# vt-asaplab/vPIN

Measured on AMD Instinct MI355X. Metric: R1CS constraints/sec, whole Spartan SNARK (sat proof + SPARK evaluation proof; vPIN point-mult + point-add instances), higher is better.
Workload: dtype u256 (integers mod q and mod p = 2^255-19, 32-bit limbs); 1 GPU; vPIN LeNet trace (layers L1..L7): 12 SNARKs per step; inputs=resident in HBM, parallelism=one trace per rank x 1 rank(s), no collective; 4 stream(s) per rank, table_slot_bytes=128

## Files before the change

### include/vpin_hip.h

```cpp
#ifndef VPIN_HIP_H
#define VPIN_HIP_H
#include <stddef.h>
#include <stdint.h>

#ifdef __cplusplus
extern "C" {
#endif

#define VPIN_OK 0
#define VPIN_EINVAL (-1)
#define VPIN_ENODEV (-2)
#define VPIN_ENOMEM (-3)
#define VPIN_EHIP (-4)
#define VPIN_ESHAPE (-5)
#define VPIN_EVERIFY (-6)

typedef struct vpin_ctx vpin_ctx;
typedef struct vpin_table vpin_table;

const char* vpin_strerror(int code);
const char* vpin_last_error(void);
int vpin_crash_line_set(const char* line, size_t n);
int vpin_abi_version(void);

// ... 559 lines not shown

int vpin_bullet_reduce(vpin_ctx* c, const vpin_gens* g, const uint8_t* x_mont, const uint8_t* a_mont, size_t R, const uint8_t* u_mont,
                       int classic, uint8_t* cLR_out, uint8_t* LR_out, uint8_t xhat_ahat_out[64], uint8_t ghat_out[32]);

int vpin_gadget_shape(int is_mult, size_t n_ops, size_t* num_cons, size_t* num_vars, size_t nnz[3]);
size_t vpin_gadget_proof_max_bytes(int is_mult, size_t n_ops);
size_t vpin_gadget_comm_bytes(int is_mult, size_t n_ops);
size_t vpin_gadget_vars_rows(int is_mult, size_t n_ops);
int vpin_host_gens_derive(const char* label, size_t nb, uint8_t* out_xyzt );
int vpin_host_merlin_kat(const char* proto, const char* label, const uint8_t* msg, size_t n, const char* clabel,
                         uint8_t* out, size_t out_n);
int vpin_host_commit(const char* label, const uint8_t* v_mont, size_t n, const uint8_t* blind_mont, uint8_t out[32]);

int vpin_host_scalar_mul2(const uint8_t a_mont[32], const uint8_t P[32], const uint8_t b_mont[32], const uint8_t Q[32], uint8_t out[32]);

int vpin_host_eq_round(const uint8_t* rand, int k, int npc, int with_dotp, int lead, const uint8_t* claims, const uint8_t* coeffs,
                       const uint8_t* res, const uint8_t* r, uint8_t* polys_out, uint8_t* state_out);

int vpin_host_mailbox_selftest(void);

#define VPIN_K_SC_CUBIC 0
#define VPIN_K_SC_QUAD 1
#define VPIN_K_SC_BIND 2
#define VPIN_K_SC_CUBIC_FUSED 3
#define VPIN_K_SC_QUAD_FUSED 4
#define VPIN_K_EQ 5
#define VPIN_K_MSM 6
#define VPIN_K_SC_TAIL 7
#define VPIN_K_SPARK_ROUND 8
#define VPIN_K_SPARK_BUILD 9
#define VPIN_K_SPARK_ROUND_BIG 10
#define VPIN_K_MSM_ROWS 11
#define VPIN_K_SPARK_TAIL 12
#define VPIN_K_COUNT 16
typedef struct {
  uint64_t launches;
  double ms;
  double alg_bytes;
  double units;
} vpin_kstat;
int vpin_prof_enable(vpin_ctx* ctx, int on);
int vpin_prof_reset(vpin_ctx* ctx);
int vpin_prof_read(vpin_ctx* ctx, vpin_kstat* stats);

#ifdef __cplusplus
}
#endif
#endif
```

### vpin_amd/capi.py

```python
import ctypes as C
import os
import re

import numpy as np

HERE = os.path.dirname(os.path.abspath(__file__))
ROOT = os.path.dirname(HERE)
HEADER = os.path.join(ROOT, "include", "vpin_hip.h")

KERNEL_CLASSES = {
    0: "sc_cubic", 1: "sc_quad", 2: "sc_bind", 3: "sc_cubic_fused", 4: "sc_quad_fused", 5: "eq", 6: "msm", 7: "sc_tail",
    8: "spark_round", 9: "spark_build", 10: "spark_round_big", 11: "msm_rows", 12: "spark_tail",
}
K_COUNT = 16


class VpinError(RuntimeError):
    def __init__(self, code, where):
        self.code = code
        L = lib()
        msg = L.vpin_strerror(code).decode()
        last = L.vpin_last_error().decode()
        super().__init__(f"{where}: {msg} ({code})" + (f" [{last}]" if last else ""))


class R1CS(C.Structure):
    _fields_ = [("num_cons", C.c_size_t), ("num_vars", C.c_size_t), ("num_inputs", C.c_size_t),
                ("nnz", C.c_size_t * 3), ("row", C.c_void_p * 3), ("col", C.c_void_p * 3), ("val", C.c_void_p * 3)]


def make_r1cs(inst):
    r = R1CS()
    r.num_cons, r.num_vars, r.num_inputs = inst["num_cons"], inst["num_vars"], inst["num_inputs"]
    keep = []
    for m, name in enumerate("ABC"):
        rows, cols, vals = (np.ascontiguousarray(x) for x in inst[name])
        keep += [rows, cols, vals]
        r.nnz[m] = len(rows)
        r.row[m] = rows.ctypes.data
        r.col[m] = cols.ctypes.data
        r.val[m] = vals.ctypes.data
    r._keep = keep
    return r


# ... 1607 lines not shown
```

### vpin_amd/csrc/host/prover_common.h

```cpp
#pragma once
#include <omp.h>

#include <chrono>
#include <cstdlib>
#include <cstring>
#include <map>
#include <memory>
#include <mutex>
#include <string>
#include <vector>

#include "../ctx.h"
#include "../comm.h"
#include "curve.h"
#include "transcript.h"

extern "C" {
size_t vpin_gens_msm_parts_count(size_t ncols);
int vpin_gens_msm_parts(vpin_ctx* ctx, const vpin_gens* g, const uint8_t* scalars_mont, size_t rows, size_t ncols,
                        uint8_t* parts_xyzt);
int vpin_poly_bound(vpin_ctx* c, const vpin_table* Z, const uint8_t* Lvec, size_t L_size, uint8_t* out_LZ);
int vpin_gens_map_stream(vpin_ctx* ctx, const uint8_t* stream64, size_t nb, uint8_t* out_xyzt);
void vpin_r1cs_dims(const vpin_r1cs_dev* d, size_t* num_cons, size_t* num_vars, size_t* num_inputs);
}
// ... 418 lines not shown
  if (fine)
    fprintf(stderr, "[dplog] R=%zu, %zu rounds, us per round: rows+inner products %.1f | host Q,H terms %.1f | wait for the MSM %.1f | "
            "sum %zu parts x2 %.1f | compress x2 + transcript + invert %.1f | fold launch %.1f\n", R, lgR, tb[0] / lgR * 1e6,
            tb[1] / lgR * 1e6, tb[2] / lgR * 1e6, np, tb[3] / lgR * 1e6, tb[4] / lgR * 1e6, tb[5] / lgR * 1e6);
  Fq xa[2];
  if (fused) rc = vpin::bullet_finish_fused(c, pc.dev, bs, B(&u_prev), B(&u_inv_prev), B(xa));
  else rc = vpin::bullet_finish(c, pc.dev, bs, B(xa), parts.data());
  if (rc) return rc;
  const Fq x_hat = xa[0], a_hat = xa[1], y_hat = x_hat * a_hat;
  Point g_hat = fused ? sum_side(0, 0) : sum_parts(parts.data());
  {
    Point p = g_hat.mul(d_);
    pc.fb_h.mul_acc(p, r_delta);
    out.delta = compress(p);
    tr.append_point("delta", out.delta.b);
    Point q = pc.fb_gR.mul(d_ * r_);
    pc.fb_h.mul_acc(q, r_beta);
    out.beta = compress(q);
    tr.append_point("beta", out.beta.b);
  }
  Fq c_ = tr.challenge_scalar("c");
  out.z1 = d_ + c_ * y_hat;
  out.z2 = a_hat * (c_ * blind_fin + r_beta) + r_delta;
  bs_guard.done = true;
  return VPIN_OK;
}

struct TableGuard {
  vpin_ctx* c;
  std::vector<vpin_table*> t;
  explicit TableGuard(vpin_ctx* c_) : c(c_) {}
  ~TableGuard() { for (auto* p : t) vpin_table_free(c, p); }
  vpin_table* add(vpin_table* p) { t.push_back(p); return p; }
};

#if defined(__clang__)
#pragma clang diagnostic pop
#endif

int sat_prove_core(vpin_ctx* c, const vpin_r1cs_dev* dinst, size_t nv, size_t ncons, size_t ni,
                   const vpin_table* d_para, const vpin_table* d_input, const vpin_table* d_vars, const uint8_t* inputs,
                   const uint8_t seed_commit64[64], const uint8_t seed_proof64[64], uint8_t* proof_out, size_t proof_cap,
                   size_t* proof_len, uint8_t* comm_para_out, uint8_t* comm_input_out, uint8_t inst_evals_out[96],
                   uint8_t* rx_out, uint8_t* ry_out, vpin_host::Transcript* tr_out, vpin_host::Transcript* tape_out);

}
```

### vpin_amd/csrc/prover.cpp

```cpp
#include "host/proof_sizes.h"
#include "host/prover_common.h"

namespace {

using namespace vpin_host;
using namespace vpin_prover;


struct SatGens {
  size_t ell = 0, L = 0, R = 0, nb = 0;
  std::vector<Point> g;
  FixedBase fb[5];
  const vpin_gens* dev = nullptr;
  PcGens pc;
  Mcg gens_1, gens_3, gens_4;
};

struct ProverCache {
  std::map<size_t, std::unique_ptr<SatGens>> by_nv;
};

static void cache_free(vpin_ctx* c) {
  auto* pc = static_cast<ProverCache*>(c->prover_cache);
  if (!pc) return;
// ... 419 lines not shown

namespace vpin_prover {

static int dist_fingerprint_check(vpin_ctx* c, size_t nv, size_t ncons, size_t ni, const uint8_t seed_commit64[64],
                                  const uint8_t seed_proof64[64]) {
  vpin_comm* cm = c->comm;
  auto fnv = [](const uint8_t* p, size_t n) { uint64_t h = 0xcbf29ce484222325ull; for (size_t i = 0; i < n; i++) { h ^= p[i]; h *= 0x100000001b3ull; } return h; };
  auto env_num = [](const char* name, long dflt) { const char* e = getenv(name); return e ? atol(e) : dflt; };
  uint64_t fp[9] = {
      (uint64_t)nv, (uint64_t)ncons, (uint64_t)ni, fnv(seed_commit64, 64), fnv(seed_proof64, 64),
      (uint64_t)(getenv("VPIN_DIST_NO_SAT_SPLIT") != nullptr), (uint64_t)(getenv("VPIN_DIST_BY_CIRCUIT") != nullptr),
      (uint64_t)env_num("VPIN_SPARK_TAIL_PAIRS", 1024), (uint64_t)(getenv("VPIN_BULLET_CLASSIC") != nullptr)};
  std::vector<uint64_t> all((size_t)cm->world * 9);
  int rc = vpin::comm_allgather_ctx(c, fp, all.data(), sizeof fp, "fingerprint");
  if (rc) return rc;
  static const char* what[9] = {"num_vars", "num_cons", "num_inputs", "seed_commit", "seed_proof", "VPIN_DIST_NO_SAT_SPLIT",
                                "VPIN_DIST_BY_CIRCUIT", "VPIN_SPARK_TAIL_PAIRS", "VPIN_BULLET_CLASSIC"};
  for (int r = 0; r < cm->world; r++)
    for (int k = 0; k < 9; k++)
      if (all[(size_t)r * 9 + k] != fp[k]) {
        char msg[200];
        snprintf(msg, sizeof msg, "collective proof: rank %d and rank %d differ in %s (%llu vs %llu)", cm->rank, r, what[k],
                 (unsigned long long)fp[k], (unsigned long long)all[(size_t)r * 9 + k]);
        vpin::set_last_error(msg, hipErrorUnknown);
        return VPIN_ECOMM;
      }
  return VPIN_OK;
}

int sat_prove_core(vpin_ctx* c, const vpin_r1cs_dev* dinst, size_t nv, size_t ncons, size_t ni,
                   const vpin_table* d_para, const vpin_table* d_input, const vpin_table* d_vars, const uint8_t* inputs,
                   const uint8_t seed_commit64[64], const uint8_t seed_proof64[64], uint8_t* proof_out, size_t proof_cap,
                   size_t* proof_len, uint8_t* comm_para_out, uint8_t* comm_input_out, uint8_t inst_evals_out[96],
                   uint8_t* rx_out, uint8_t* ry_out, vpin_host::Transcript* tr_out, vpin_host::Transcript* tape_out) {
  auto t_begin = Clock::now();
  memset(g_timings, 0, sizeof g_timings);
  (void)hipSetDevice(c->device);

  SatGens* sg = nullptr;
  auto t0 = Clock::now();
  int rc = get_gens(c, nv, &sg);
  if (rc) return rc;
  g_timings[5] = secs(t0, Clock::now());
  const size_t L = sg->L, R = sg->R;
  TableGuard tg(c);

  t0 = Clock::now();
  vpin_comm* cm = (c->comm && c->comm->world > 1) ? c->comm : nullptr;
  if (cm && (rc = dist_fingerprint_check(c, nv, ncons, ni, seed_commit64, seed_proof64))) return rc;
  const size_t nrows = cm ? vpin::comm_strided_count(L, cm->rank, cm->world) : L;
  vpin::CommitPairState* cps = nullptr;
  if (nrows && (rc = vpin::commit_pair_begin(c, sg->dev, d_para, d_input, L, &cps, cm ? (size_t)cm->rank : 0, nrows, cm ? (size_t)cm->world : 1)))
    return rc;
  const uint8_t two = 2;
  Transcript tape1 = make_tape(&two, 1, seed_commit64);
  std::vector<Fq> blind_para = tape1.challenge_vector("poly_blinds", L);
  std::vector<Fq> blind_input = tape1.challenge_vector("poly_blinds", L);
  std::vector<Fq> blind_vars(L);
  for (size_t i = 0; i < L; i++) blind_vars[i] = blind_para[i] + blind_input[i];
  std::vector<CG> comm_vars(L);
  if (!cm) {
    rc = vpin::commit_pair_finish(c, sg->dev, cps, B(blind_para.data()), B(blind_input.data()), R + 1, comm_para_out,
                                  comm_input_out, comm_vars[0].b);
    if (rc) return rc;
  } else {
    const size_t pmax = vpin::comm_block_max(L, cm->world);
    std::vector<uint8_t> mine(3 * pmax * 32, 0), all((size_t)cm->world * 3 * pmax * 32);
// ... 57 lines not shown
  vpin_table* tabs1[3] = {d_abc[0], d_abc[1], d_abc[2]};
  rc = zk_sumcheck(c, 4, tabs1, Fq::zero(), Fq::zero(), nrx, sg->gens_1, sg->gens_4, tr, tape, sc1, rx, claims1, blind_post1,
                   &tau, d_pyr, lw);
  if (rc) return rc;
  if ((rc = vpin::comm_mark(c, "sat_phase1_rest"))) return rc;
  vpin::ctx_enter_alt(c);
  if (c->progress_flag) *c->progress_flag = 1;
  g_timings[1] = secs(t0, Clock::now());

  const Fq tau_claim = claims1[0], Az_claim = claims1[1], Bz_claim = claims1[2], Cz_claim = claims1[3];
  Fq Az_blind = tape.challenge_scalar("Az_blind"), Bz_blind = tape.challenge_scalar("Bz_blind"),
     Cz_blind = tape.challenge_scalar("Cz_blind"), prod_blind = tape.challenge_scalar("prod_Az_Bz_blind");
  KnowProof pok_Cz;
  CG comm_Cz = knowledge_prove(pok_Cz, sg->gens_1, tr, tape, Cz_claim, Cz_blind);
  ProdProof pprod;
  CG comm_Az, comm_Bz, comm_prod;
  product_prove(pprod, sg->gens_1, tr, tape, Az_claim, Az_blind, Bz_claim, Bz_blind, Az_claim * Bz_claim, prod_blind, comm_Az,
                comm_Bz, comm_prod);
  tr.append_point("comm_Az_claim", comm_Az.b);
  tr.append_point("comm_Bz_claim", comm_Bz.b);
  tr.append_point("comm_Cz_claim", comm_Cz.b);
  tr.append_point("comm_prod_Az_Bz_claims", comm_prod.b);
  Fq blind_expected1 = tau_claim * (prod_blind - Cz_blind);
  Fq claim_post1 = (Az_claim * Bz_claim - Cz_claim) * tau_claim;
  EqProof eq1;
  equality_prove(eq1, sg->gens_1, tr, tape, claim_post1, blind_expected1, claim_post1, blind_post1);

  t0 = Clock::now();
  Fq r_A = tr.challenge_scalar("challenege_Az"), r_B = tr.challenge_scalar("challenege_Bz"),
     r_C = tr.challenge_scalar("challenege_Cz");
  Fq claim2 = r_A * Az_claim + r_B * Bz_claim + r_C * Cz_claim;
  Fq blind_claim2 = r_A * Az_blind + r_B * Bz_blind + r_C * Cz_blind;
  vpin_table *d_eq_rx = nullptr, *d_eabc = nullptr;
  if ((rc = vpin_eq_table(c, B(rx.data()), nrx, &d_eq_rx))) return rc;
  tg.add(d_eq_rx);
  t_spmv = Clock::now();
  {
    Fq rabc[3] = {r_A, r_B, r_C};
    if (lw) rc = vpin::r1cs_eval_table_strided(c, dinst, d_eq_rx, B(rabc), wrank, wstep, &d_eabc);
    else rc = vpin_r1cs_eval_table(c, dinst, d_eq_rx, B(rabc), &d_eabc);
    if (rc) return rc;
    tg.add(d_eabc);
  }
  g_timings[6] += secs(t_spmv, Clock::now());
  Fq claims2[2], blind_post2;
  vpin_table* d_z2 = d_z;
  if (lw) {
    if ((rc = vpin::table_take_strided(c, d_z, wrank, wstep, &d_z2))) return rc;
    tg.add(d_z2);
  }
  vpin_table* tabs2[2] = {d_z2, d_eabc};
  rc = zk_sumcheck(c, 2, tabs2, claim2, blind_claim2, nry, sg->gens_1, sg->gens_3, tr, tape, sc2, ry, claims2, blind_post2, nullptr,
                   nullptr, lw);
  if (rc) return rc;
  if ((rc = vpin::comm_mark(c, "sat_phase2_rest"))) return rc;
  g_timings[2] = secs(t0, Clock::now());

  t0 = Clock::now();
  const size_t left = sg->ell / 2, right = sg->ell - left;
  std::vector<Fq> Lv(L), Rv(R), LZ(R);
  host_eq(ry.data() + 1, left, Lv.data());
  host_eq(ry.data() + 1 + left, right, Rv.data());
  if (cm) rc = vpin::poly_bound_dist(c, d_vars, B(Lv.data()), L, B(LZ.data()));
  else rc = vpin_poly_bound(c, d_vars, B(Lv.data()), L, B(LZ.data()));
  if (rc) return rc;
  Fq eval_vars_at_ry = Fq::zero();
  for (size_t i = 0; i < R; i++) eval_vars_at_ry = eval_vars_at_ry + LZ[i] * Rv[i];
  Fq blind_eval = tape.challenge_scalar("blind_eval");
  tr.append_protocol_name("polynomial evaluation proof");
  Fq LZ_blind = Fq::zero();
  for (size_t i = 0; i < L; i++) LZ_blind = LZ_blind + blind_vars[i] * Lv[i];

  DpLog pe;
  if ((rc = dplog_prove(c, sg->pc, tr, tape, LZ, LZ_blind, Rv, eval_vars_at_ry, blind_eval, pe))) return rc;
  g_timings[3] = secs(t0, Clock::now());

  Fq blind_eval_Z = (one - ry[0]) * blind_eval;
  Fq blind_expected2 = claims2[1] * blind_eval_Z;
  Fq claim_post2 = claims2[0] * claims2[1];
  EqProof eq2;
  equality_prove(eq2, sg->gens_1, tr, tape, claim_post2, blind_expected2, claim_post2, blind_post2);

  t0 = Clock::now();
  Fq ie[3];
  {
    vpin_table* d_eq_ry = nullptr;
    if ((rc = vpin_eq_table(c, B(ry.data()), nry, &d_eq_ry))) return rc;
    tg.add(d_eq_ry);
    if ((rc = vpin_r1cs_evaluate(c, dinst, d_eq_rx, d_eq_ry, B(ie)))) return rc;
  }
  tr.append_scalar("Ar_claim", ie[0]);
  tr.append_scalar("Br_claim", ie[1]);
  tr.append_scalar("Cr_claim", ie[2]);
  memcpy(inst_evals_out, ie, 96);
  g_timings[7] = secs(t0, Clock::now());

  Writer w;
  w.u64(L);
  for (auto& cg : comm_vars) w.point(cg);
  write_zksc(w, sc1);
  w.point(comm_Az); w.point(comm_Bz); w.point(comm_Cz); w.point(comm_prod);
  w.point(pok_Cz.alpha); w.scalar(pok_Cz.z1); w.scalar(pok_Cz.z2);
  w.point(pprod.alpha); w.point(pprod.beta); w.point(pprod.delta);
  for (int i = 0; i < 5; i++) w.scalar(pprod.z[i]);
  w.point(eq1.alpha); w.scalar(eq1.z);
  write_zksc(w, sc2);
  w.point(pe.Cy);
  write_dplog(w, pe);
  w.point(eq2.alpha); w.scalar(eq2.z);
  if (w.buf.size() > proof_cap) return VPIN_ESHAPE;
  memcpy(proof_out, w.buf.data(), w.buf.size());
  *proof_len = w.buf.size();
  if (rx_out) memcpy(rx_out, rx.data(), rx.size() * 32);
  if (ry_out) memcpy(ry_out, ry.data(), ry.size() * 32);
  if ((rc = vpin::comm_mark(c, "sat_replicated"))) return rc;
  if (tr_out) *tr_out = tr;
  if (tape_out) *tape_out = tape;
  g_timings[4] = secs(t_begin, Clock::now());
// ... 83 lines not shown
```

### vpin_amd/csrc/r1cs.hip

```cpp
#include <algorithm>
#include <cstring>
#include <vector>

#include "ctx.h"
#include "r1cs_dev.h"

namespace vpin {

constexpr int kRB = 256;

__device__ __forceinline__ fq mul_special(const fq& val, const fq& x) {
  return fq_mul(val, x);
}

__global__ __launch_bounds__(kRB) void spmv_kernel(const uint32_t* __restrict__ rowptr, const uint32_t* __restrict__ col,
                                                   const fq* __restrict__ val, const fq* __restrict__ z, size_t nrows,
                                                   fq* __restrict__ out) {
  size_t r = (size_t)blockIdx.x * kRB + threadIdx.x;
  if (r >= nrows) return;
  uint32_t k0 = rowptr[r], k1 = rowptr[r + 1];
  fq acc = fq_zero();
  for (uint32_t k = k0; k < k1; k++) {
    fq x = fq_load(z + col[k]);
    if (fq_is_zero(x)) continue;
// ... 557 lines not shown
    if (d->n_long[m]) {
      hipLaunchKernelGGL(long_chunk_kernel, dim3((unsigned)d->n_chunks[m]), dim3(kRB), 0, c->stream, d->chunk_k0[m],
                         d->chunk_k1[m], d->csc_row[m], d->csc_val[m], evals_rx->d, chunk_partials);
      hipLaunchKernelGGL(eval_table_long_finish_strided_kernel, dim3((unsigned)d->n_long[m]), dim3(64), 0, c->stream,
                         d->long_cols[m], d->long_first[m], d->n_long[m], chunk_partials, rc_m, r0, step, t->d);
    }
  }
  hipError_t e = hipGetLastError();
  if (e != hipSuccess) { set_last_error("eval_table_strided", e); vpin_table_free(c, t); return VPIN_EHIP; }
  *out = t;
  return VPIN_OK;
}

}

extern "C" {

int vpin_r1cs_evaluate(vpin_ctx* c, const vpin_r1cs_dev* d, const vpin_table* evals_rx, const vpin_table* evals_ry,
                       uint8_t out[96]) {
  if (!c || !d || !evals_rx || !evals_ry || !out) return VPIN_EINVAL;
  if (evals_rx->len != d->num_cons || evals_ry->len != 2 * d->num_vars) return VPIN_ESHAPE;
  (void)hipSetDevice(c->device);
  const size_t ncols = 2 * d->num_vars;
  DevBuf bo(c), chunk_scratch(c);
  if (bo.alloc(96)) return VPIN_ENOMEM;
  fq* d_out = (fq*)bo.p;
  const size_t max_chunks = std::max(d->n_chunks[0], std::max(d->n_chunks[1], d->n_chunks[2]));
  if (max_chunks && chunk_scratch.alloc(max_chunks * sizeof(fq))) return VPIN_ENOMEM;
  fq* chunk_partials = (fq*)chunk_scratch.p;
  int grid = (int)std::min<size_t>((ncols + kRB - 1) / kRB, 1024);
  for (int m = 0; m < 3; m++) {
    int nparts = grid + (int)d->n_long[m];
    if ((size_t)nparts > c->partials_cap) return VPIN_ESHAPE;
    hipLaunchKernelGGL(evaluate_kernel, dim3(grid), dim3(kRB), 0, c->stream, d->colptr[m], d->csc_row[m], d->csc_val[m],
                       evals_rx->d, evals_ry->d, ncols, c->d_partials);
    if (d->n_long[m]) {
      hipLaunchKernelGGL(long_chunk_kernel, dim3((unsigned)d->n_chunks[m]), dim3(kRB), 0, c->stream, d->chunk_k0[m],
                         d->chunk_k1[m], d->csc_row[m], d->csc_val[m], evals_rx->d, chunk_partials);
      hipLaunchKernelGGL(evaluate_long_finish_kernel, dim3((unsigned)d->n_long[m]), dim3(64), 0, c->stream,
                         d->long_cols[m], d->long_first[m], d->n_long[m], chunk_partials, evals_ry->d, c->d_partials + grid);
    }
    hipLaunchKernelGGL(sum_partials_kernel, dim3(1), dim3(kRB), 0, c->stream, c->d_partials, nparts, d_out + m);
  }
  hipError_t e = hipGetLastError();
  if (e == hipSuccess) e = hipMemcpyAsync(out, d_out, 96, hipMemcpyDeviceToHost, c->stream);
  if (e == hipSuccess) e = hipStreamSynchronize(c->stream);
  if (e != hipSuccess) { set_last_error("vpin_r1cs_evaluate", e); return VPIN_EHIP; }
  return VPIN_OK;
}

}
```

### vpin_amd/csrc/spark.cpp

```cpp
#include <cstdio>

#include "host/proof_sizes.h"
#include "host/prover_common.h"
#include "gadget_dev.h"
#include "spark_dev.h"

namespace {

using namespace vpin_host;
using namespace vpin_prover;

static bool spark_trace() { static const bool on = getenv("VPIN_SPARK_TRACE") != nullptr; return on; }
struct TraceSpan {
  const char* name; Clock::time_point t0;
  explicit TraceSpan(const char* n) : name(n), t0(Clock::now()) {}
  ~TraceSpan() { if (spark_trace()) fprintf(stderr, "[spark] %-28s %8.3f ms\n", name, secs(t0, Clock::now()) * 1e3); }
};


struct SparkGens {
  std::vector<Point> g;
  std::map<size_t, std::unique_ptr<PcGens>> views;
};

// ... 595 lines not shown
}

struct SparkProof {
  vpin_ctx* c;
  const vpin_spark_decomm* d;
  const std::vector<Fq>&rx, &ry;
  const Fq* evals;
  Transcript &tr, &tape;
  const size_t N, M, lgN, lgM;
  const PcGens *g_ops = nullptr, *g_mem = nullptr, *g_derefs = nullptr;
  TableGuard tg;
  DistPlan plan;
  const DistPlan* dz = nullptr;
  bool st = false;
  vpin::SparkLeaves leaves;
  size_t Nf = 0, Mf = 0;
  bool defer_mem = false;
  vpin_table *mem_rx = nullptr, *mem_ry = nullptr, *comb = nullptr;
  vpin_table comb_shape;
  vpin::DevBuf b_cloc, b_crows, b_vloc, b_ops, b_mem, b_scr;
  vpin::fq* comb_rows = nullptr;
  const vpin::fq *derefs = nullptr, *vals = nullptr;
  std::vector<CG> comm_derefs;
  vpin::HashParams hash;
  vpin::SparkForest f_ops, f_mem;
  Fq pl[2][8];
  DotpCtx dotp;
  Fq dotp_left[3], dotp_right[3];
  Batched pf_ops, pf_mem;
  std::vector<Fq> rand_ops, rand_mem;
  Fq ev_derefs[6], ev_ops[15], ev_mem[2];
  DpLog pe_derefs, pe_ops, pe_mem;

  SparkProof(vpin_ctx* c_, const vpin_spark_decomm* d_, const std::vector<Fq>& rx_, const std::vector<Fq>& ry_, const Fq* evals_,
             Transcript& tr_, Transcript& tape_)
      : c(c_), d(d_), rx(rx_), ry(ry_), evals(evals_), tr(tr_), tape(tape_), N(d_->N), M(d_->M), lgN(log2z(d_->N)), lgM(log2z(d_->M)),
        tg(c_), b_cloc(c_), b_crows(c_), b_vloc(c_), b_ops(c_), b_mem(c_), b_scr(c_) {}
  bool by_circuit() const { return dz && !st; }
};

static int split_plan(SparkProof& S) {
  vpin_ctx* c = S.c;
  if (!(c->comm && c->comm->world > 1)) return VPIN_OK;
  if (c->comm->world > 12) return VPIN_EINVAL;
  plan_init(S.plan, c->comm);
  S.dz = &S.plan;
  static const bool by_circuit = getenv("VPIN_DIST_BY_CIRCUIT") != nullptr;
  const size_t Wz = (size_t)S.plan.world;
  if (!by_circuit && (Wz & (Wz - 1)) == 0 && Wz <= 16 && S.N / Wz >= 4096 && S.M / Wz >= 4096 && S.g_derefs->L >= Wz)
    S.plan.lw = (int)log2z(Wz);
  S.st = S.plan.lw > 0;
  if (S.st) { S.leaves.r0 = (size_t)S.plan.rank; S.leaves.step = Wz; }
  return VPIN_OK;
}

static int stage_derefs(SparkProof& S) {
  vpin_ctx* c = S.c;
  const vpin_spark_decomm* d = S.d;
  const DistPlan* dz = S.dz;
  const PcGens* g_derefs = S.g_derefs;
  const size_t N = S.N;
  int rc;
  S.tr.append_protocol_name("Sparse polynomial evaluation proof");
  const size_t nm = std::max(d->nx, d->ny);
  std::vector<Fq> rx_ext(nm, Fq::zero()), ry_ext(nm, Fq::zero());
  std::copy(S.rx.begin(), S.rx.end(), rx_ext.begin() + (nm - d->nx));
  std::copy(S.ry.begin(), S.ry.end(), ry_ext.begin() + (nm - d->ny));
  if ((rc = vpin_eq_table(c, B(rx_ext.data()), (int)nm, &S.mem_rx))) return rc;
  S.tg.add(S.mem_rx);
  if ((rc = vpin_eq_table(c, B(ry_ext.data()), (int)nm, &S.mem_ry))) return rc;
  S.tg.add(S.mem_ry);
  const vpin::fq *mem_rx = S.mem_rx->d, *mem_ry = S.mem_ry->d;
  S.Nf = N / S.leaves.step; S.Mf = S.M / S.leaves.step;
  if (S.st) {
    S.comb_shape.d = nullptr; S.comb_shape.len = S.comb_shape.cap = 8 * N; S.comb_shape.owned = false;
    S.comb = &S.comb_shape;
    const size_t Nl = S.Nf, nrows_loc = vpin::comm_strided_count(g_derefs->L, dz->rank, dz->world);
    if (S.b_cloc.alloc(6 * Nl * 32) || S.b_crows.alloc(std::max<size_t>(1, nrows_loc) * g_derefs->R * 32) || S.b_vloc.alloc(3 * Nl * 32)) return VPIN_ENOMEM;
    S.comb_rows = (vpin::fq*)S.b_crows.p;
    if ((rc = vpin::spark_gather_derefs(c, d, S.leaves, mem_rx, mem_ry, (vpin::fq*)S.b_cloc.p, S.comb_rows, g_derefs->R, nrows_loc))) return rc;
    for (int m = 0; m < 3; m++)
      if ((rc = vpin::spark_take_strided(c, d->vals + (size_t)m * N, Nl, S.leaves.r0, S.leaves.step, (vpin::fq*)S.b_vloc.p + (size_t)m * Nl))) return rc;
    S.derefs = (const vpin::fq*)S.b_cloc.p; S.vals = (const vpin::fq*)S.b_vloc.p;
  } else {
    if ((rc = vpin::table_alloc_uninit(c, 8 * N, &S.comb))) return rc;
    S.tg.add(S.comb);
    if ((rc = vpin::spark_gather_derefs(c, d, S.leaves, mem_rx, mem_ry, S.comb->d))) return rc;
    S.derefs = S.comb->d; S.vals = d->vals;
  }
  if ((rc = vpin::comm_mark(c, "derefs_gather"))) return rc;
  std::vector<CG>& comm_derefs = S.comm_derefs;
  const bool hot = d->hot_col[0] != 0xffffffffu || d->hot_col[1] != 0xffffffffu || d->hot_col[2] != 0xffffffffu;
  const uint32_t* col_idx[3] = {d->idx + 6 * N, d->idx + 7 * N, d->idx + 8 * N};
  if (dz) {
    const size_t L = g_derefs->L, pmax = vpin::comm_block_max(L, dz->world);
    const size_t nrows = vpin::comm_strided_count(L, dz->rank, dz->world);
    std::vector<uint8_t> mine(pmax * 32, 0), all(pmax * 32 * (size_t)dz->world);
    if (nrows) {
      if (hot)
        rc = vpin::hyrax_commit_derefs_hot(c, g_derefs->dev, S.comb, L, N, col_idx, d->hot_col, mem_ry, mine.data(), (size_t)dz->rank,
                                           nrows, (size_t)dz->world, S.comb_rows);
      else
        rc = vpin::hyrax_commit_rows_strided(c, g_derefs->dev, S.comb, L, (size_t)dz->rank, nrows, (size_t)dz->world, mine.data(), S.comb_rows);
      if (rc) return rc;
    }
    if ((rc = vpin::comm_allgather_ctx(c, mine.data(), all.data(), mine.size(), "derefs_commit"))) return rc;
    comm_derefs.resize(L);
    for (int r = 0; r < dz->world; r++) {
      const size_t n = vpin::comm_strided_count(L, r, dz->world);
      for (size_t k = 0; k < n; k++) memcpy(comm_derefs[(size_t)r + k * (size_t)dz->world].b, all.data() + ((size_t)r * pmax + k) * 32, 32);
    }
  } else if (hot) {
    comm_derefs.resize(g_derefs->L);
    if ((rc = vpin::hyrax_commit_derefs_hot(c, g_derefs->dev, S.comb, g_derefs->L, N, col_idx, d->hot_col, mem_ry, comm_derefs[0].b))) return rc;
  } else if ((rc = commit_noblind(c, g_derefs, S.comb, comm_derefs))) {
    return rc;
  }
  S.tr.append_message("derefs_commitment", "begin_derefs_commitment");
  append_polycomm(S.tr, "comm_poly_row_col_ops_val", comm_derefs);
  S.tr.append_message("derefs_commitment", "end_derefs_commitment");
  return VPIN_OK;
}

// ... 76 lines not shown
      if (S.defer_mem) {
        if ((rc = vpin::spark_mem_roots(c, S.d, S.hash, S.mem_rx->d, S.mem_ry->d))) return rc;
      } else if (S.f_mem.ncirc && (rc = vpin::spark_fetch_tops(c, &S.f_mem, 2))) {
        return rc;
      }
      t = reinterpret_cast<const Fq*>(c->h_spark);
      if (dz) {
        if ((rc = dist_exchange(c, *dz, true, false, t, 2, roots.data(), "roots"))) return rc;
        t = roots.data();
      }
    }
    for (int s = 0; s < 2; s++) { pl[s][0] = t[2 * (2 * s)]; pl[s][7] = t[2 * (2 * s + 1)]; }
  }
  static const char* lab[2][4] = {{"claim_row_eval_init", "claim_row_eval_read", "claim_row_eval_write", "claim_row_eval_audit"},
                                  {"claim_col_eval_init", "claim_col_eval_read", "claim_col_eval_write", "claim_col_eval_audit"}};
  for (int s = 0; s < 2; s++) {
    Fq ws = Fq::one(), rs = Fq::one();
    for (int m = 0; m < 3; m++) { rs = rs * pl[s][1 + m]; ws = ws * pl[s][4 + m]; }
    if (!(pl[s][0] * ws == rs * pl[s][7])) return VPIN_ESHAPE;
    S.tr.append_scalar(lab[s][0], pl[s][0]);
    S.tr.append_scalars(lab[s][1], &pl[s][1], 3);
    S.tr.append_scalars(lab[s][2], &pl[s][4], 3);
    S.tr.append_scalar(lab[s][3], pl[s][7]);
  }
  return VPIN_OK;
}

static int dotp_claims(SparkProof& S) {
  vpin_ctx* c = S.c;
  const DistPlan* dz = S.dz;
  int rc;
  const std::vector<int>* hv = S.by_circuit() ? &dz->dotp_of[dz->rank] : nullptr;
  const size_t nh = hv ? hv->size() : 6;
  if (nh && (rc = vpin::spark_triple_sums(c, S.derefs, S.vals, S.Nf, hv ? hv->data() : nullptr, (int)nh))) return rc;
  Fq mine6[6] = {};
  for (size_t i = 0; i < nh; i++) mine6[hv ? (*hv)[i] : i] = reinterpret_cast<const Fq*>(c->h_spark)[3 * i];
  if (S.st) rc = dist_sum(c, *dz, mine6, 6, S.dotp.claims, "triple_sums");
  else if (dz) rc = dist_pick(c, *dz, mine6, 6, dz->owner_dotp, S.dotp.claims, "triple_sums");
  else std::copy(mine6, mine6 + 6, S.dotp.claims);
  if (rc) return rc;
  for (int m = 0; m < 3; m++) {
    S.dotp_left[m] = S.dotp.claims[2 * m];
    S.dotp_right[m] = S.dotp.claims[2 * m + 1];
    S.tr.append_scalar("claim_eval_dotp_left", S.dotp_left[m]);
    S.tr.append_scalar("claim_eval_dotp_right", S.dotp_right[m]);
    if (!(S.dotp_left[m] + S.dotp_right[m] == S.evals[m])) return VPIN_ESHAPE;
  }
  return VPIN_OK;
}

static int stage_product(SparkProof& S) {
  vpin_ctx* c = S.c;
  int rc;
  S.tr.append_protocol_name("Sparse polynomial evaluation proof");
  S.tr.append_protocol_name("Sparse polynomial product layer proof");
  if ((rc = product_roots(S))) return rc;
  S.dotp = DotpCtx{S.d, S.Nf, S.vals, S.derefs, (vpin::fq*)S.b_scr.p, {}};
  if ((rc = dotp_claims(S))) return rc;
  {
    TraceSpan ts("product: ops forest");
    if ((rc = product_prove(c, S.f_ops, 12, &S.dotp, S.tr, S.pf_ops, S.rand_ops, S.dz))) return rc;
  }
  if (S.defer_mem) {
    TraceSpan ts("network: mem forest (deferred)");
    S.b_ops.release();
    S.b_scr.release();
    if (S.b_mem.alloc((size_t)4 * 2 * S.M * 32)) return VPIN_ENOMEM;
    S.f_mem.base = (vpin::fq*)S.b_mem.p;
    if ((rc = vpin::spark_build_forest(c, S.d, S.hash, S.leaves, {nullptr, S.mem_rx->d, S.mem_ry->d}, &S.f_mem, true))) return rc;
// ... 130 lines not shown
    if ((rc = vpin::spark_slice_evals(c, comb_ops->d, N, 15, eq_ops->d))) return rc;
    for (int i = 0; i < 15; i++) S.ev_ops[i] = hs[3 * i];
    if ((rc = vpin::spark_slice_evals(c, comb_mem->d, M, 2, eq_mem->d))) return rc;
    for (int i = 0; i < 2; i++) S.ev_mem[i] = hs[3 * i];
  }
  std::vector<Fq> e16(16, Fq::zero());
  std::copy(S.ev_ops, S.ev_ops + 15, e16.begin());
  if ((rc = prove_joint(S, *S.g_ops, comb_ops, sp_ops, e16, 4, rand_ops,
                        {"claim_evals_ops", "challenge_combine_n_to_one", "joint_claim_eval_ops", "hash: polyeval ops"}, nullptr, S.pe_ops)))
    return rc;
  return prove_joint(S, *S.g_mem, comb_mem, sp_mem, {S.ev_mem[0], S.ev_mem[1]}, 1, rand_mem,
                     {"claim_evals_mem", "challenge_combine_two_to_one", "joint_claim_eval_mem", "hash: polyeval mem"}, nullptr, S.pe_mem);
}

static void write_proof(const SparkProof& S, Writer& w) {
  const auto& pl = S.pl;
  w.u64(S.comm_derefs.size());
  for (auto& p : S.comm_derefs) w.point(p);
  for (int s = 0; s < 2; s++) { w.scalar(pl[s][0]); w_scalars(w, &pl[s][1], 3); w_scalars(w, &pl[s][4], 3); w.scalar(pl[s][7]); }
  w_scalars(w, S.dotp_left, 3);
  w_scalars(w, S.dotp_right, 3);
  write_batched(w, S.pf_mem);
  write_batched(w, S.pf_ops);
  w_scalars(w, &S.ev_ops[0], 3); w_scalars(w, &S.ev_ops[3], 3); w.scalar(S.ev_mem[0]);
  w_scalars(w, &S.ev_ops[6], 3); w_scalars(w, &S.ev_ops[9], 3); w.scalar(S.ev_mem[1]);
  w_scalars(w, &S.ev_ops[12], 3);
  w_scalars(w, &S.ev_derefs[0], 3); w_scalars(w, &S.ev_derefs[3], 3);
  write_dplog(w, S.pe_ops);
  write_dplog(w, S.pe_mem);
  write_dplog(w, S.pe_derefs);
}

static int spark_prove(vpin_ctx* c, const vpin_spark_decomm* d, const std::vector<Fq>& rx, const std::vector<Fq>& ry,
                       const Fq evals[3], Transcript& tr, Transcript& tape, Writer& w) {
  if (d->N < 4 || d->M < 4 || rx.size() != d->nx || ry.size() != d->ny) return VPIN_ESHAPE;
  int rc;
  SparkProof S(c, d, rx, ry, evals, tr, tape);
  const Shape sh{d->nx, d->ny, S.N, S.M, S.lgN + 4, std::max(d->nx, d->ny) + 1, S.lgN + 3};
  if ((rc = get_view(c, std::max(sh.v_ops, sh.v_mem), &S.g_ops)) || (rc = get_view(c, sh.v_ops, &S.g_ops)) ||
      (rc = get_view(c, sh.v_mem, &S.g_mem)) || (rc = get_view(c, sh.v_derefs, &S.g_derefs)))
    return rc;
  auto t0 = Clock::now();
  auto lap = [&](int slot) { g_spark_timings[slot] = secs(t0, Clock::now()); t0 = Clock::now(); };
  if ((rc = split_plan(S)) || (rc = stage_derefs(S))) return rc;
  lap(1);
  if (c->progress_flag) *c->progress_flag = 2;
  if ((rc = stage_network(S))) return rc;
  lap(2);
  if ((rc = stage_product(S))) return rc;
  lap(3);
  if ((rc = stage_hash(S))) return rc;
  lap(4);
  write_proof(S, w);
  return VPIN_OK;
}

}

extern "C" {

size_t vpin_spark_comm_bytes(const vpin_r1cs* inst) {
  return inst ? vpin_sizes::spark_comm_bytes(inst->num_cons, inst->num_vars, inst->nnz) : 0;
}

size_t vpin_snark_proof_max_bytes(const vpin_r1cs* inst) {
  return inst ? vpin_sizes::snark_proof_max_bytes(inst->num_cons, inst->num_vars, inst->nnz) : 0;
}

int vpin_spark_prepare(vpin_ctx* c, size_t num_cons, size_t num_vars, size_t max_nnz) {
  if (!c || !vpin::is_pow2(num_cons) || !vpin::is_pow2(num_vars) || max_nnz == 0) return VPIN_EINVAL;
  (void)hipSetDevice(c->device);
  const size_t nnz[3] = {max_nnz, max_nnz, max_nnz};
  const Shape s = shape_of(num_cons, num_vars, nnz);
  const PcGens* g = nullptr;
  int rc = get_view(c, std::max(s.v_ops, s.v_mem), &g);
  if (!rc) {
    auto* sg = static_cast<SparkGens*>(c->spark_cache);
    std::vector<size_t> idx;
    for (size_t ell : {s.v_ops, s.v_mem, s.v_derefs}) {
      const size_t R = (size_t)1 << (ell - ell / 2);
      if (R + 1 < sg->g.size()) { idx.push_back(R); idx.push_back(R + 1); }
    }
#pragma omp parallel for schedule(dynamic, 1) num_threads(host_threads())
    for (long k = 0; k < (long)idx.size(); k++) { FixedBase warm(sg->g[idx[(size_t)k]]); (void)warm; }
  }
  if (!rc) rc = get_view(c, s.v_ops, &g);
// ... 199 lines not shown
  memcpy(rand.data(), r, r_len * 32);
  SlicePass sp(c);
  std::vector<Fq> ev((size_t)used);
  int rc = sp.run(c, pc, (const uint32_t*)b32.p, n32, used > n32 ? Zfq->d : nullptr, nbits, used, rand, ev.data());
  if (rc) return rc;
  memcpy(evals_out, ev.data(), (size_t)used * 32);
  if (ch && LZ_out) {
    std::vector<Fq> chv((size_t)nbits), LZ;
    memcpy(chv.data(), ch, (size_t)nbits * 32);
    if ((rc = sp.combine(c, pc, chv, LZ))) return rc;
    memcpy(LZ_out, LZ.data(), pc.R * 32);
  }
  return VPIN_OK;
}

int vpin_snark_prove_resident(vpin_ctx* c, const vpin_r1cs_dev* dinst, const vpin_spark_decomm* decomm,
                              const vpin_table* vars_para, const vpin_table* vars_input, const vpin_table* vars,
                              const uint8_t* inputs, const uint8_t seed_commit64[64], const uint8_t seed_proof64[64],
                              uint8_t* proof_out, size_t proof_cap, size_t* proof_len, uint8_t* comm_para_out,
                              uint8_t* comm_input_out) {
  if (!c || !dinst || !decomm || !vars_para || !vars_input || !vars || !seed_commit64 || !seed_proof64 || !proof_out ||
      !proof_len || !comm_para_out || !comm_input_out)
    return VPIN_EINVAL;
  size_t nv, ncons, ni;
  vpin_r1cs_dims(dinst, &ncons, &nv, &ni);
  if (vars_para->len != nv || vars_input->len != nv || vars->len != nv || (ni && !inputs)) return VPIN_ESHAPE;
  if (decomm->num_cons != ncons || decomm->num_vars != nv || decomm->num_inputs != ni) return VPIN_ESHAPE;
  auto t0 = Clock::now();
  vpin::AltStreamGuard alt_guard(c);
  Transcript tr("snark_example"), tape("snark_example");
  uint8_t ie[96];
  std::vector<Fq> rx(log2z(ncons)), ry(log2z(2 * nv));
  size_t sat_len = 0;
  int rc = sat_prove_core(c, dinst, nv, ncons, ni, vars_para, vars_input, vars, inputs, seed_commit64, seed_proof64, proof_out,
                          proof_cap, &sat_len, comm_para_out, comm_input_out, ie, B(rx.data()), B(ry.data()), &tr, &tape);
  if (rc) return vpin::comm_leave(c->comm, rc);
  if (c->progress_flag) *c->progress_flag = 1;
  g_spark_timings[5] = secs(t0, Clock::now());
  Writer w;
  w.bytes(ie, 96);
  Fq evals[3];
  memcpy(evals, ie, 96);
  if ((rc = spark_prove(c, decomm, rx, ry, evals, tr, tape, w))) return vpin::comm_leave(c->comm, rc);
  if (sat_len + w.buf.size() > proof_cap) return VPIN_ESHAPE;
  memcpy(proof_out + sat_len, w.buf.data(), w.buf.size());
  *proof_len = sat_len + w.buf.size();
  g_spark_timings[6] = secs(t0, Clock::now());
  return VPIN_OK;
}

int vpin_snark_prove(vpin_ctx* c, const vpin_r1cs* inst, const uint8_t* vars_para, const uint8_t* vars_input,
                     const uint8_t* vars, const uint8_t* inputs, const uint8_t seed_commit64[64], const uint8_t seed_proof64[64],
                     uint8_t* proof_out, size_t proof_cap, size_t* proof_len, uint8_t* comm_out, size_t comm_cap, size_t* comm_len,
                     uint8_t* comm_para_out, uint8_t* comm_input_out) {
  if (!c || !inst || !vars_para || !vars_input || !vars) return VPIN_EINVAL;
  const size_t nv = inst->num_vars;
  if (!vpin::is_pow2(nv) || !vpin::is_pow2(inst->num_cons) || inst->num_inputs >= nv) return VPIN_ESHAPE;
  vpin_r1cs_dev* dinst = nullptr;
  vpin_spark_decomm* decomm = nullptr;
  const bool trace = getenv("VPIN_CLI_TRACE") != nullptr;
  auto t0 = std::chrono::steady_clock::now();
  auto lap = [&](const char* what) {
    if (!trace) return;
    (void)hipStreamSynchronize(c->stream);
    auto t1 = std::chrono::steady_clock::now();
    fprintf(stderr, "[vpin_snark_prove] %-18s %9.1f ms\n", what, std::chrono::duration<double, std::milli>(t1 - t0).count());
    t0 = t1;
  };
  int rc = vpin_r1cs_upload(c, inst, &dinst);
  if (rc) return rc;
  lap("r1cs_upload");
  TableGuard tg(c);
  vpin_table *d_para = nullptr, *d_input = nullptr, *d_vars = nullptr;
  rc = vpin_spark_encode(c, inst, &decomm, comm_out, comm_cap, comm_len);
  lap("spark_encode");
  if (!rc) rc = vpin_table_upload(c, vars_para, nv, &d_para);
// ... 34 lines not shown
```

Before: 78.19 million constraints/s.

## Compute inst evals via SPARK deref gather, reusing eq tables across sat and SPARK

```diff
diff --git a/include/vpin_hip.h b/include/vpin_hip.h
--- a/include/vpin_hip.h
+++ b/include/vpin_hip.h
@@ -615,6 +615,7 @@
 #define VPIN_K_SPARK_ROUND_BIG 10
 #define VPIN_K_MSM_ROWS 11
 #define VPIN_K_SPARK_TAIL 12
+#define VPIN_K_R1CS_EVALUATE 13
 #define VPIN_K_COUNT 16
 typedef struct {
   uint64_t launches;
diff --git a/vpin_amd/capi.py b/vpin_amd/capi.py
--- a/vpin_amd/capi.py
+++ b/vpin_amd/capi.py
@@ -11,6 +11,7 @@
 KERNEL_CLASSES = {
     0: "sc_cubic", 1: "sc_quad", 2: "sc_bind", 3: "sc_cubic_fused", 4: "sc_quad_fused", 5: "eq", 6: "msm", 7: "sc_tail",
     8: "spark_round", 9: "spark_build", 10: "spark_round_big", 11: "msm_rows", 12: "spark_tail",
+    13: "r1cs_evaluate",
 }
 K_COUNT = 16
 
diff --git a/vpin_amd/csrc/host/prover_common.h b/vpin_amd/csrc/host/prover_common.h
--- a/vpin_amd/csrc/host/prover_common.h
+++ b/vpin_amd/csrc/host/prover_common.h
@@ -474,7 +474,21 @@
   explicit TableGuard(vpin_ctx* c_) : c(c_) {}
   ~TableGuard() { for (auto* p : t) vpin_table_free(c, p); }
   vpin_table* add(vpin_table* p) { t.push_back(p); return p; }
+  void release_all_but(vpin_table* keep) {
+    for (auto* p : t)
+      if (p != keep) vpin_table_free(c, p);
+    t.clear();
+  }
 };
+
+struct SparkPrelude {
+  const vpin_spark_decomm* d = nullptr;
+  vpin_table *mem_rx = nullptr, *mem_ry = nullptr, *comb = nullptr;
+  Fq sums[6];
+  bool done = false;
+  size_t nm() const;
+};
+int spark_prelude(vpin_ctx* c, SparkPrelude& P, const std::vector<Fq>& rx, const std::vector<Fq>& ry, vpin_table* eq_rx);
 
 #if defined(__clang__)
 #pragma clang diagnostic pop
@@ -484,6 +498,7 @@
                    const vpin_table* d_para, const vpin_table* d_input, const vpin_table* d_vars, const uint8_t* inputs,
                    const uint8_t seed_commit64[64], const uint8_t seed_proof64[64], uint8_t* proof_out, size_t proof_cap,
                    size_t* proof_len, uint8_t* comm_para_out, uint8_t* comm_input_out, uint8_t inst_evals_out[96],
-                   uint8_t* rx_out, uint8_t* ry_out, vpin_host::Transcript* tr_out, vpin_host::Transcript* tape_out);
-
-}
+                   uint8_t* rx_out, uint8_t* ry_out, vpin_host::Transcript* tr_out, vpin_host::Transcript* tape_out,
+                   SparkPrelude* pre = nullptr);
+
+}
diff --git a/vpin_amd/csrc/prover.cpp b/vpin_amd/csrc/prover.cpp
--- a/vpin_amd/csrc/prover.cpp
+++ b/vpin_amd/csrc/prover.cpp
@@ -475,7 +475,8 @@
                    const vpin_table* d_para, const vpin_table* d_input, const vpin_table* d_vars, const uint8_t* inputs,
                    const uint8_t seed_commit64[64], const uint8_t seed_proof64[64], uint8_t* proof_out, size_t proof_cap,
                    size_t* proof_len, uint8_t* comm_para_out, uint8_t* comm_input_out, uint8_t inst_evals_out[96],
-                   uint8_t* rx_out, uint8_t* ry_out, vpin_host::Transcript* tr_out, vpin_host::Transcript* tape_out) {
+                   uint8_t* rx_out, uint8_t* ry_out, vpin_host::Transcript* tr_out, vpin_host::Transcript* tape_out,
+                   SparkPrelude* pre) {
   auto t_begin = Clock::now();
   memset(g_timings, 0, sizeof g_timings);
   (void)hipSetDevice(c->device);
@@ -599,8 +600,21 @@
   Fq claim2 = r_A * Az_claim + r_B * Bz_claim + r_C * Cz_claim;
   Fq blind_claim2 = r_A * Az_blind + r_B * Bz_blind + r_C * Cz_blind;
   vpin_table *d_eq_rx = nullptr, *d_eabc = nullptr;
-  if ((rc = vpin_eq_table(c, B(rx.data()), nrx, &d_eq_rx))) return rc;
-  tg.add(d_eq_rx);
+  if (pre && (cm || c->low_memory || getenv("VPIN_MEM_FOREST_LATE"))) pre = nullptr;
+  vpin_table* d_eq_rx_ext = nullptr;
+  vpin_table eq_rx_view;
+  if (pre && pre->nm() > (size_t)nrx) {
+    std::vector<Fq> rx_ext(pre->nm(), Fq::zero());
+    std::copy(rx.begin(), rx.end(), rx_ext.begin() + (pre->nm() - (size_t)nrx));
+    if ((rc = vpin_eq_table(c, B(rx_ext.data()), (int)pre->nm(), &d_eq_rx_ext))) return rc;
+    tg.add(d_eq_rx_ext);
+    eq_rx_view.d = d_eq_rx_ext->d; eq_rx_view.len = eq_rx_view.cap = (size_t)1 << nrx; eq_rx_view.owned = false;
+    d_eq_rx = &eq_rx_view;
+  } else {
+    if ((rc = vpin_eq_table(c, B(rx.data()), nrx, &d_eq_rx))) return rc;
+    tg.add(d_eq_rx);
+    if (pre) d_eq_rx_ext = d_eq_rx;
+  }
   t_spmv = Clock::now();
   {
     Fq rabc[3] = {r_A, r_B, r_C};
@@ -650,7 +664,11 @@
 
   t0 = Clock::now();
   Fq ie[3];
-  {
+  if (pre) {
+    tg.release_all_but(d_eq_rx_ext);
+    if ((rc = spark_prelude(c, *pre, rx, ry, d_eq_rx_ext))) return rc;
+    for (int m = 0; m < 3; m++) ie[m] = pre->sums[2 * m] + pre->sums[2 * m + 1];
+  } else {
     vpin_table* d_eq_ry = nullptr;
     if ((rc = vpin_eq_table(c, B(ry.data()), nry, &d_eq_ry))) return rc;
     tg.add(d_eq_ry);
diff --git a/vpin_amd/csrc/r1cs.hip b/vpin_amd/csrc/r1cs.hip
--- a/vpin_amd/csrc/r1cs.hip
+++ b/vpin_amd/csrc/r1cs.hip
@@ -613,8 +613,11 @@
   for (int m = 0; m < 3; m++) {
     int nparts = grid + (int)d->n_long[m];
     if ((size_t)nparts > c->partials_cap) return VPIN_ESHAPE;
-    hipLaunchKernelGGL(evaluate_kernel, dim3(grid), dim3(kRB), 0, c->stream, d->colptr[m], d->csc_row[m], d->csc_val[m],
-                       evals_rx->d, evals_ry->d, ncols, c->d_partials);
+    {
+      ProfScope ps(c, VPIN_K_R1CS_EVALUATE, (double)d->nnz[m] * 68.0 + (double)ncols * 36.0);
+      hipLaunchKernelGGL(evaluate_kernel, dim3(grid), dim3(kRB), 0, c->stream, d->colptr[m], d->csc_row[m], d->csc_val[m],
+                         evals_rx->d, evals_ry->d, ncols, c->d_partials);
+    }
     if (d->n_long[m]) {
       hipLaunchKernelGGL(long_chunk_kernel, dim3((unsigned)d->n_chunks[m]), dim3(kRB), 0, c->stream, d->chunk_k0[m],
                          d->chunk_k1[m], d->csc_row[m], d->csc_val[m], evals_rx->d, chunk_partials);
diff --git a/vpin_amd/csrc/spark.cpp b/vpin_amd/csrc/spark.cpp
--- a/vpin_amd/csrc/spark.cpp
+++ b/vpin_amd/csrc/spark.cpp
@@ -651,6 +651,7 @@
   Fq ev_derefs[6], ev_ops[15], ev_mem[2];
   DpLog pe_derefs, pe_ops, pe_mem;
 
+  SparkPrelude* pre = nullptr;
   SparkProof(vpin_ctx* c_, const vpin_spark_decomm* d_, const std::vector<Fq>& rx_, const std::vector<Fq>& ry_, const Fq* evals_,
              Transcript& tr_, Transcript& tape_)
       : c(c_), d(d_), rx(rx_), ry(ry_), evals(evals_), tr(tr_), tape(tape_), N(d_->N), M(d_->M), lgN(log2z(d_->N)), lgM(log2z(d_->M)),
@@ -673,6 +674,8 @@
   return VPIN_OK;
 }
 
+static int commit_derefs(SparkProof& S);
+
 static int stage_derefs(SparkProof& S) {
   vpin_ctx* c = S.c;
   const vpin_spark_decomm* d = S.d;
@@ -681,6 +684,14 @@
   const size_t N = S.N;
   int rc;
   S.tr.append_protocol_name("Sparse polynomial evaluation proof");
+  S.Nf = N / S.leaves.step; S.Mf = S.M / S.leaves.step;
+  if (S.pre) {
+    SparkPrelude& P = *S.pre;
+    S.mem_rx = S.tg.add(P.mem_rx); S.mem_ry = S.tg.add(P.mem_ry); S.comb = S.tg.add(P.comb);
+    P.mem_rx = P.mem_ry = P.comb = nullptr;
+    S.derefs = S.comb->d; S.vals = d->vals;
+    return commit_derefs(S);
+  }
   const size_t nm = std::max(d->nx, d->ny);
   std::vector<Fq> rx_ext(nm, Fq::zero()), ry_ext(nm, Fq::zero());
   std::copy(S.rx.begin(), S.rx.end(), rx_ext.begin() + (nm - d->nx));
@@ -690,7 +701,6 @@
   if ((rc = vpin_eq_table(c, B(ry_ext.data()), (int)nm, &S.mem_ry))) return rc;
   S.tg.add(S.mem_ry);
   const vpin::fq *mem_rx = S.mem_rx->d, *mem_ry = S.mem_ry->d;
-  S.Nf = N / S.leaves.step; S.Mf = S.M / S.leaves.step;
   if (S.st) {
     S.comb_shape.d = nullptr; S.comb_shape.len = S.comb_shape.cap = 8 * N; S.comb_shape.owned = false;
     S.comb = &S.comb_shape;
@@ -708,6 +718,17 @@
     S.derefs = S.comb->d; S.vals = d->vals;
   }
   if ((rc = vpin::comm_mark(c, "derefs_gather"))) return rc;
+  return commit_derefs(S);
+}
+
+static int commit_derefs(SparkProof& S) {
+  vpin_ctx* c = S.c;
+  const vpin_spark_decomm* d = S.d;
+  const DistPlan* dz = S.dz;
+  const PcGens* g_derefs = S.g_derefs;
+  const size_t N = S.N;
+  const vpin::fq* mem_ry = S.mem_ry->d;
+  int rc;
   std::vector<CG>& comm_derefs = S.comm_derefs;
   const bool hot = d->hot_col[0] != 0xffffffffu || d->hot_col[1] != 0xffffffffu || d->hot_col[2] != 0xffffffffu;
   const uint32_t* col_idx[3] = {d->idx + 6 * N, d->idx + 7 * N, d->idx + 8 * N};
@@ -850,9 +871,13 @@
   int rc;
   const std::vector<int>* hv = S.by_circuit() ? &dz->dotp_of[dz->rank] : nullptr;
   const size_t nh = hv ? hv->size() : 6;
-  if (nh && (rc = vpin::spark_triple_sums(c, S.derefs, S.vals, S.Nf, hv ? hv->data() : nullptr, (int)nh))) return rc;
   Fq mine6[6] = {};
-  for (size_t i = 0; i < nh; i++) mine6[hv ? (*hv)[i] : i] = reinterpret_cast<const Fq*>(c->h_spark)[3 * i];
+  if (S.pre) {
+    std::copy(S.pre->sums, S.pre->sums + 6, mine6);
+  } else {
+    if (nh && (rc = vpin::spark_triple_sums(c, S.derefs, S.vals, S.Nf, hv ? hv->data() : nullptr, (int)nh))) return rc;
+    for (size_t i = 0; i < nh; i++) mine6[hv ? (*hv)[i] : i] = reinterpret_cast<const Fq*>(c->h_spark)[3 * i];
+  }
   if (S.st) rc = dist_sum(c, *dz, mine6, 6, S.dotp.claims, "triple_sums");
   else if (dz) rc = dist_pick(c, *dz, mine6, 6, dz->owner_dotp, S.dotp.claims, "triple_sums");
   else std::copy(mine6, mine6 + 6, S.dotp.claims);
@@ -1049,10 +1074,11 @@
 }
 
 static int spark_prove(vpin_ctx* c, const vpin_spark_decomm* d, const std::vector<Fq>& rx, const std::vector<Fq>& ry,
-                       const Fq evals[3], Transcript& tr, Transcript& tape, Writer& w) {
+                       const Fq evals[3], Transcript& tr, Transcript& tape, Writer& w, SparkPrelude* pre) {
   if (d->N < 4 || d->M < 4 || rx.size() != d->nx || ry.size() != d->ny) return VPIN_ESHAPE;
   int rc;
   SparkProof S(c, d, rx, ry, evals, tr, tape);
+  if (pre && pre->done) S.pre = pre;
   const Shape sh{d->nx, d->ny, S.N, S.M, S.lgN + 4, std::max(d->nx, d->ny) + 1, S.lgN + 3};
   if ((rc = get_view(c, std::max(sh.v_ops, sh.v_mem), &S.g_ops)) || (rc = get_view(c, sh.v_ops, &S.g_ops)) ||
       (rc = get_view(c, sh.v_mem, &S.g_mem)) || (rc = get_view(c, sh.v_derefs, &S.g_derefs)))
@@ -1069,6 +1095,36 @@
   if ((rc = stage_hash(S))) return rc;
   lap(4);
   write_proof(S, w);
+  return VPIN_OK;
+}
+
+}
+
+namespace vpin_prover {
+
+size_t SparkPrelude::nm() const { return std::max(d->nx, d->ny); }
+
+int spark_prelude(vpin_ctx* c, SparkPrelude& P, const std::vector<Fq>& rx, const std::vector<Fq>& ry, vpin_table* eq_rx) {
+  const vpin_spark_decomm* d = P.d;
+  P.mem_rx = eq_rx;
+  if (d->N < 4 || d->M < 4 || rx.size() != d->nx || ry.size() != d->ny) return VPIN_ESHAPE;
+  const size_t nm = P.nm();
+  int rc;
+  if (!P.mem_rx) {
+    std::vector<Fq> rx_ext(nm, Fq::zero());
+    std::copy(rx.begin(), rx.end(), rx_ext.begin() + (nm - d->nx));
+    if ((rc = vpin_eq_table(c, B(rx_ext.data()), (int)nm, &P.mem_rx))) return rc;
+  } else if (P.mem_rx->len != ((size_t)1 << nm)) {
+    return VPIN_ESHAPE;
+  }
+  std::vector<Fq> ry_ext(nm, Fq::zero());
+  std::copy(ry.begin(), ry.end(), ry_ext.begin() + (nm - d->ny));
+  if ((rc = vpin_eq_table(c, B(ry_ext.data()), (int)nm, &P.mem_ry))) return rc;
+  if ((rc = vpin::table_alloc_uninit(c, 8 * d->N, &P.comb))) return rc;
+  if ((rc = vpin::spark_gather_derefs(c, d, vpin::SparkLeaves{}, P.mem_rx->d, P.mem_ry->d, P.comb->d))) return rc;
+  if ((rc = vpin::spark_triple_sums(c, P.comb->d, d->vals, d->N))) return rc;
+  for (int i = 0; i < 6; i++) P.sums[i] = reinterpret_cast<const Fq*>(c->h_spark)[3 * i];
+  P.done = true;
   return VPIN_OK;
 }
 
@@ -1334,8 +1390,14 @@
   uint8_t ie[96];
   std::vector<Fq> rx(log2z(ncons)), ry(log2z(2 * nv));
   size_t sat_len = 0;
+  SparkPrelude pre;
+  pre.d = decomm;
+  struct PreGuard {
+    vpin_ctx* c; SparkPrelude& p;
+    ~PreGuard() { for (vpin_table* t : {p.mem_rx, p.mem_ry, p.comb}) if (t) vpin_table_free(c, t); }
+  } pre_guard{c, pre};
   int rc = sat_prove_core(c, dinst, nv, ncons, ni, vars_para, vars_input, vars, inputs, seed_commit64, seed_proof64, proof_out,
-                          proof_cap, &sat_len, comm_para_out, comm_input_out, ie, B(rx.data()), B(ry.data()), &tr, &tape);
+                          proof_cap, &sat_len, comm_para_out, comm_input_out, ie, B(rx.data()), B(ry.data()), &tr, &tape, &pre);
   if (rc) return vpin::comm_leave(c->comm, rc);
   if (c->progress_flag) *c->progress_flag = 1;
   g_spark_timings[5] = secs(t0, Clock::now());
@@ -1343,7 +1405,7 @@
   w.bytes(ie, 96);
   Fq evals[3];
   memcpy(evals, ie, 96);
-  if ((rc = spark_prove(c, decomm, rx, ry, evals, tr, tape, w))) return vpin::comm_leave(c->comm, rc);
+  if ((rc = spark_prove(c, decomm, rx, ry, evals, tr, tape, w, &pre))) return vpin::comm_leave(c->comm, rc);
   if (sat_len + w.buf.size() > proof_cap) return VPIN_ESHAPE;
   memcpy(proof_out + sat_len, w.buf.data(), w.buf.size());
   *proof_len = sat_len + w.buf.size();
```

Result: no change. 78.69 million constraints/s, median of 6 (+0.6%).
